# aalto-speech/AaltoASR

Measured on AMD Instinct MI355X. Metric: frames/sec GMM log-lik (39-d, 50k Gauss) + MFCC, 1/2/4/8 MI355X, higher is better.
Workload: dtype f32 (2-term fp16 split on the matrix cores, f32 accumulate); 1 GPU; configs[2]: full MFCC chain (FFT -> mel -> log -> DCT -> delta/delta-delta, CMS, normalisation) + 50000-Gaussian scoring + 2-byte LNA codes on 1 h of synthetic 16 kHz audio as 360 x 10 s utterances (449280 frames), int16 samples resident in HBM; dim=39, gaussians=50000, states=3125, gpus_flag=1

## Files before the change

### aaltoasr_amd/capi.py

```python
from __future__ import annotations

import ctypes as C
import os
import re
from typing import Optional

import numpy as np

HERE = os.path.dirname(os.path.abspath(__file__))
LIB_PATH = os.path.join(os.environ.get("AASR_LIBDIR") or os.path.join(HERE, "lib"), "libaasr.so")
HEADER_PATH = os.path.join(HERE, "..", "include", "aasr.h")

AASR_OK = 0
AASR_ERR_INVALID = -1
AASR_ERR_UNSUPPORTED = -2
AASR_ERR_NO_DEVICE = -3
AASR_ERR_IO = -4
AASR_ERR_SHORT_AUDIO = -5


class AasrError(RuntimeError):
    def __init__(self, code: int, msg: str):
        super().__init__("aasr status %d: %s" % (code, msg))
        self.code = code
# ... 596 lines not shown
        out = np.empty((n_frames, dim), dtype)
        fn = lib().aasr_feat_run if dtype == np.float32 else lib().aasr_feat_run_f64
        check(fn(self._h, _ptr(pcm), len(pcm), first_frame, n_frames,
                 module.encode() if module else None, _ptr(out)))
        return out

    def run_features(self, frames: np.ndarray, first_frame: int, n_frames: int,
                     module: Optional[str] = None, dtype=np.float32) -> np.ndarray:
        frames = np.ascontiguousarray(frames, np.float32)
        dim = self.module_dim(module) if module else self.dim
        out = np.empty((n_frames, dim), dtype)
        fn = lib().aasr_feat_run_features if dtype == np.float32 else lib().aasr_feat_run_features_f64
        check(fn(self._h, _ptr(frames), frames.size, first_frame, n_frames,
                 module.encode() if module else None, _ptr(out)))
        return out

    def run_batch_dev(self, d_pcm, pcm_off: np.ndarray, frame_off: np.ndarray, d_out, stream=None):
        pcm_off = np.ascontiguousarray(pcm_off, np.int64)
        frame_off = np.ascontiguousarray(frame_off, np.int64)
        check(lib().aasr_feat_run_batch_dev(self._h, _ptr(d_pcm), _ptr(pcm_off), _ptr(frame_off),
                                            len(pcm_off) - 1, _ptr(d_out), _stream_handle(stream)))

    def set_parameters(self, module: str, block_text: str) -> None:
        check(lib().aasr_feat_set_parameters(self._h, module.encode(), block_text.encode()))

    def get_parameters(self, module: str) -> str:
        out = C.c_void_p()
        n = C.c_int64()
        check(lib().aasr_feat_get_parameters(self._h, module.encode(), C.byref(out), C.byref(n)))
        try:
            return C.string_at(out, n.value).decode()
        finally:
            lib().aasr_free(out)

    def modules(self):
        L = lib()
        return [(L.aasr_feat_module_name(self._h, i).decode(), L.aasr_feat_module_type(self._h, i).decode())
                for i in range(L.aasr_feat_num_modules(self._h))]


def recipe_batch_range(total: int, num_batches: int, batch_index: int):
    f, n = C.c_int32(), C.c_int32()
    check(lib().aasr_recipe_batch_range(total, num_batches, batch_index, C.byref(f), C.byref(n)))
    return f.value, n.value


def debug_feat_fusion(on: bool) -> None:
    L = lib()
    L.aasr_debug_feat_fusion.argtypes = [C.c_int]
    L.aasr_debug_feat_fusion.restype = None
    L.aasr_debug_feat_fusion(int(on))


def debug_cluster_heap(on: bool) -> None:
    L = lib()
    L.aasr_debug_cluster_heap.argtypes = [C.c_int]
    L.aasr_debug_cluster_heap.restype = None
    L.aasr_debug_cluster_heap(int(on))


def recipe_frame_limits(start_time: float, end_time: float, frame_rate: float):
    a, b = C.c_int32(), C.c_int32()
    lib().aasr_recipe_frame_limits(start_time, end_time, frame_rate, C.byref(a), C.byref(b))
    return a.value, b.value


def recipe_read(text, num_batches: int = 0, batch_index: int = 0):
    out = C.c_void_p()
    n = C.c_int64()
    raw = text if isinstance(text, bytes) else text.encode()
    check(lib().aasr_recipe_read(raw, num_batches, batch_index, C.byref(out), C.byref(n)))
    try:
        table = C.string_at(out, n.value)
    finally:
        lib().aasr_free(out)
    rows = []
    for line in table.split(b"\n")[:-1]:
        f = line.split(b"\x1f")
        rows.append(tuple(x.decode("latin-1") for x in f[:4]) +
                    (float(np.float32(float(f[4]))), float(np.float32(float(f[5])))))
    return rows


def recipe_read_all(text, num_batches: int = 0, batch_index: int = 0, cluster_speakers: bool = False):
    out = C.c_void_p()
    n = C.c_int64()
    raw = text if isinstance(text, bytes) else text.encode()
    check(lib().aasr_recipe_read_all(raw, num_batches, batch_index, int(cluster_speakers), C.byref(out), C.byref(n)))
    try:
        table = C.string_at(out, n.value)
    finally:
        lib().aasr_free(out)
    rows = []
    for line in table.split(b"\n")[:-1]:
        f = [x.decode("latin-1") for x in line.split(b"\x1f")]
        rows.append(tuple(f[:7]) + (float(np.float32(float(f[7]))), float(np.float32(float(f[8]))),
                                    int(f[9]), int(f[10]), f[11], f[12]))
    return rows


def lna_read_file(path: str):
    out = C.POINTER(C.c_float)()
    S = C.c_int32()
    nb = C.c_int32()
    F = C.c_int64()
    check(lib().aasr_lna_read_file(path.encode(), C.byref(S), C.byref(nb), C.byref(F), C.byref(out)))
# ... 548 lines not shown
```

### aaltoasr_amd/csrc/feat_kernels.hip

```cpp
#include <hip/hip_runtime.h>

#include <cmath>
#include <cstring>
#include <climits>

#include "feat.h"

namespace aasr {

struct DevBatch {
  int n_utts;
  const int64_t *frame_off;
  const int64_t *pcm_off;
  const int32_t *first;
  const int32_t *eof_frame;
};

__device__ __forceinline__ int find_utt(const DevBatch &b, int64_t r, int span) {
  int lo = 0, hi = b.n_utts - 1;
  while (lo < hi) {
    int mid = (lo + hi + 1) >> 1;
    int64_t key = b.frame_off[mid] + (int64_t)mid * span;
    if (key <= r) lo = mid; else hi = mid - 1;
  }
  return lo;
}

__device__ __forceinline__ int find_utt_near(const DevBatch &b, int64_t r, int span, int64_t rows) {
  const int n = b.n_utts;
  int u = (int)((float)r * (float)n / (float)rows);
  u = u < 0 ? 0 : (u > n - 1 ? n - 1 : u);
  int lo = 0, hi = n - 1;
  for (int step = 0; step < 3; step++) {
    const int64_t k0 = b.frame_off[u] + (int64_t)u * span;
    const int64_t k1 = b.frame_off[u + 1] + (int64_t)(u + 1) * span;
    if (k0 > r && u > 0) {
      hi = u - 1;
      u--;
    } else if (k1 <= r && u < n - 1) {
      lo = u + 1;
      u++;
    } else {
      return u;
    }
  }
  while (lo < hi) {
    int mid = (lo + hi + 1) >> 1;
    int64_t key = b.frame_off[mid] + (int64_t)mid * span;
    if (key <= r) lo = mid; else hi = mid - 1;
  }
  return lo;
}

struct SrcMap {
// ... 188 lines not shown
  for (int q1 = 0, k = u; q1 < pr; q1++, k += m) scratch[q1] = F[k];
  for (int q1 = 0, k = u; q1 < pr; q1++, k += m) {
    int twidx = 0;
    cpx acc = scratch[0];
    for (int q = 1; q < pr; q++) {
      twidx += fstride * k;
      if (twidx >= n) twidx -= n;
      const cpx t = cmul(scratch[q], tw[twidx]);
      acc.r += t.r;
      acc.i += t.i;
    }
    F[k] = acc;
  }
}

__device__ __forceinline__ float glibc_logf(float x) {
  const double T[16][2] = {
      {0x1.661ec79f8f3bep+0, -0x1.57bf7808caadep-2}, {0x1.571ed4aaf883dp+0, -0x1.2bef0a7c06ddbp-2},
      {0x1.49539f0f010bp+0, -0x1.01eae7f513a67p-2},  {0x1.3c995b0b80385p+0, -0x1.b31d8a68224e9p-3},
      {0x1.30d190c8864a5p+0, -0x1.6574f0ac07758p-3}, {0x1.25e227b0b8eap+0, -0x1.1aa2bc79c81p-3},
      {0x1.1bb4a4a1a343fp+0, -0x1.a4e76ce8c0e5ep-4}, {0x1.12358f08ae5bap+0, -0x1.1973c5a611cccp-4},
      {0x1.0953f419900a7p+0, -0x1.252f438e10c1ep-5}, {0x1p+0, 0x0p+0},
      {0x1.e608cfd9a47acp-1, 0x1.aa5aa5df25984p-5},  {0x1.ca4b31f026aap-1, 0x1.c5e53aa362eb4p-4},
      {0x1.b2036576afce6p-1, 0x1.526e57720db08p-3},  {0x1.9c2d163a1aa2dp-1, 0x1.bc2860d22477p-3},
      {0x1.886e6037841edp-1, 0x1.1058bc8a07ee1p-2},  {0x1.767dcf5534862p-1, 0x1.4043057b6ee09p-2}};
  const double Ln2 = 0x1.62e42fefa39efp-1;
  const double A0 = -0x1.00ea348b88334p-2, A1 = 0x1.5575b0be00b6ap-2, A2 = -0x1.ffffef20a4123p-2;
  const uint32_t ix = __float_as_uint(x);
  if (ix == 0x3f800000u) return 0.0f;
  if (ix - 0x00800000u >= 0x7f800000u - 0x00800000u) return (float)log((double)x);
  const uint32_t tmp = ix - 0x3f330000u;
  const int i = (int)((tmp >> 19) & 15u);
  const int k = (int32_t)tmp >> 23;
  const uint32_t iz = ix - (tmp & 0xff800000u);
  const double z = (double)__uint_as_float(iz);
  const double r = z * T[i][0] - 1.0;
  const double y0 = T[i][1] + (double)k * Ln2;
  const double r2 = r * r;
  double y = A1 * r + A2;
  y = A0 * r2 + y;
  y = y * r2 + (y0 + r);
  return (float)y;
}

__device__ __forceinline__ float spec_value(float re, float im, int magnitude, int take_log) {
  float a = re * re;
  float c = im * im;
  float v = a + c;
  if (magnitude) v = (float)sqrt((double)v);
  if (take_log) v = glibc_logf(v);
  return v;
}

__device__ __forceinline__ void real_split(const cpx *buf, int nc, int k, const cpx *__restrict__ stw,
                                           float &re_k, float &im_k, float &re_n, float &im_n) {
  cpx fpk = buf[k], fpnk, f1k, f2k, t;
  fpnk.r = buf[nc - k].r;
  fpnk.i = -buf[nc - k].i;
  f1k.r = fpk.r + fpnk.r;  f1k.i = fpk.i + fpnk.i;
  f2k.r = fpk.r - fpnk.r;  f2k.i = fpk.i - fpnk.i;
  t = cmul(f2k, stw[k - 1]);
  float ar = f1k.r + t.r, ai = f1k.i + t.i, br = f1k.r - t.r, bi = t.i - f1k.i;
  re_k = ar * .5f;
  im_k = ai * .5f;
  re_n = br * .5f;
  im_n = bi * .5f;
}

template <bool FROM_PCM, bool GEN>
__global__ __launch_bounds__(256) void k_fft(DevBatch b, const int16_t *__restrict__ pcm,
                                             AudioPrm ap, const double *__restrict__ src,
                                             SrcMap sm, int L, int R, int64_t rows, FftPrm fp,
                                             double *__restrict__ dst) {
  extern __shared__ __attribute__((aligned(16))) char smem_raw[];
  const int wave = threadIdx.x >> 6, lane = threadIdx.x & 63;
  const int64_t r = (int64_t)blockIdx.x * 4 + wave;
  if (r >= rows) return;
  cpx *buf = (cpx *)smem_raw + (size_t)wave * fp.nc;
  const int nc = fp.nc, width = 2 * nc;

  const int16_t *p = nullptr;
  int64_t nsamp = 0, ws = 0;
  const double *xrow = nullptr;
  if (FROM_PCM) {
    int u = find_utt(b, r, L + R);
    int frame = b.first[u] - L + (int)(r - (b.frame_off[u] + (int64_t)u * (L + R)));
    ws = window_start(b, u, frame, ap);
    p = pcm + b.pcm_off[u];
    nsamp = b.pcm_off[u + 1] - b.pcm_off[u];
  } else {
    xrow = src + src_row(b, r, L + R, sm) * width;
  }
  for (int o = lane; o < nc; o += 64) {
    int s = fp.perm[o];
    double x0, x1;
    if (FROM_PCM) {
      x0 = (double)preemph_sample(p, nsamp, ws + 2 * s, ap.emph);
      x1 = (double)preemph_sample(p, nsamp, ws + 2 * s + 1, ap.emph);
    } else {
      x0 = xrow[2 * s];
      x1 = xrow[2 * s + 1];
    }
    cpx v;
    v.r = (float)((double)fp.hamming[2 * s] * x0);
    v.i = (float)((double)fp.hamming[2 * s + 1] * x1);
    buf[o] = v;
  }
  __builtin_amdgcn_fence(__ATOMIC_RELEASE, "wavefront");
  __builtin_amdgcn_wave_barrier();

  const cpx *tw = (const cpx *)fp.twiddle;
  for (int s = fp.ns - 1; s >= 0; s--) {
    const int pr = fp.radix[s], m = fp.sublen[s];
    const int fstride = fp.fstride[s];
    const int nb = fstride * m;
    if (GEN && pr > 5) {
      for (int bi = lane; bi < nb; bi += 64) kiss_butterfly_generic(buf, bi, pr, m, fstride, tw);
    } else {
      for (int bi = lane; bi < nb; bi += 64) kiss_butterfly(buf, bi, pr, m, fp.sub_magic[s], fstride, tw);
// ... 203 lines not shown
        power = power + v0;
        power = power + v1;
        power = power + v2;
        power = power + v3;
        power = power + v4;
        power = power + v5;
        power = power + v6;
        power = power + v7;
      }
      for (; i < nbins; i++) power = power + sf[i];
      if (r0 + ff < rows && !AASR_FDBG(128)) dst[(r0 + ff) * out_dim + sp.dct_dim] = log((double)power + 1e-10);
    }
    for (int slot = l; slot < (AASR_FDBG(4) ? 0 : sp.mel_dim); slot += TPF) {
      const int bin = t_mord[slot];
      float val = 0;
      const int e_end = t_moff[bin + 1];
      int e = t_moff[bin];
      for (; e + 4 <= e_end; e += 4) {
        const double p0 = (double)t_msc[e] * (double)spec[t_mt[e]];
        const double p1 = (double)t_msc[e + 1] * (double)spec[t_mt[e + 1]];
        const double p2 = (double)t_msc[e + 2] * (double)spec[t_mt[e + 2]];
        const double p3 = (double)t_msc[e + 3] * (double)spec[t_mt[e + 3]];
        val = (float)((double)val + p0);
        val = (float)((double)val + p1);
        val = (float)((double)val + p2);
        val = (float)((double)val + p3);
      }
      for (; e < e_end; e++) val = (float)((double)val + (double)t_msc[e] * (double)spec[t_mt[e]]);
      const float q = (float)((double)val / (double)t_msum[bin]);
      double o;
      if (sp.mel_root) {
        o = pow((double)q, 0.1);
      } else {
        const float a = q + 1.0f;
        o = (double)glibc_logf(a);
      }
      melv[(size_t)f * sp.mel_dim + bin] = o;
    }
    __builtin_amdgcn_fence(__ATOMIC_RELEASE, "wavefront");
    __builtin_amdgcn_wave_barrier();
    if (r0 + f < rows && !AASR_FDBG(128)) {
      const double *data = melv + (size_t)f * sp.mel_dim;
      for (int i = l; i < sp.dct_dim; i += TPF) {
        double acc = 0.0;
        if (sp.zeroth && i == 0) {
          for (int k = 0; k < sp.mel_dim; k++) acc += data[k];
        } else {
          const spec_tbl_t *c = t_dct + (size_t)(i - (sp.zeroth ? 1 : 0)) * sp.mel_dim;
#pragma unroll 4
          for (int k = 0; k < sp.mel_dim; k++) acc += data[k] * (double)c[k];
        }
        dst[(r0 + f) * out_dim + i] = acc;
      }
    }
    __builtin_amdgcn_fence(__ATOMIC_RELEASE, "wavefront");
    __builtin_amdgcn_wave_barrier();
  }
}

struct TemporalPrm {
  int dx, w1, w2;
  float norm1, norm2;
  const float *mean, *scale;
  const float *matrix, *bias;
  int dim;
};

#ifdef AASR_TR
constexpr int kTemporalRows = AASR_TR;
#else
constexpr int kTemporalRows = 64;
#endif

static inline size_t temporal_smem(int tile_rows, int dx, int H, int w2, int dim) {
  return (size_t)(tile_rows + 2 * H) * dx * 8 + (size_t)(tile_rows + 2 * w2) * dx * 8 + (size_t)tile_rows * 3 * dx * 8 + 16 +
         (size_t)(3 * dx) * ((dim + 2) / 3) * 16 + (size_t)(6 * dx + dim) * 4;
}

template <int ROWS, int NT>
__global__ __launch_bounds__(NT) void k_temporal_fused(DevBatch b, const double *__restrict__ src,
                                                        SrcMap sm, int span, int64_t rows,
                                                        TemporalPrm tp, int dbg, double *__restrict__ dst) {
  extern __shared__ __attribute__((aligned(16))) char smem_raw[];
  const int dx = tp.dx, H = tp.w1 + tp.w2, md = 3 * tp.dx;
  const unsigned dx_magic = fast_magic(dx), dim_magic = fast_magic(tp.dim);
  double *xs = (double *)smem_raw;
  double *d1 = xs + (size_t)(ROWS + 2 * H) * dx;
  double *nrm = d1 + (size_t)(ROWS + 2 * tp.w2) * dx;
  float4 *mt = (float4 *)(smem_raw + ((((size_t)(2 * ROWS + 2 * H + 2 * tp.w2) * dx + (size_t)ROWS * md) * 8 + 15) & ~(size_t)15));
  const int ngrp = (tp.dim + 2) / 3;
  const unsigned ngrp_magic = fast_magic(ngrp);
  if (tp.matrix && !AASR_FDBG(8))
    for (int e = threadIdx.x; e < md * ngrp; e += NT) {
      const int j = fast_div(e, ngrp_magic), g = e - j * ngrp;
      float4 v;
      v.x = tp.matrix[(size_t)(3 * g) * md + j];
      v.y = 3 * g + 1 < tp.dim ? tp.matrix[(size_t)(3 * g + 1) * md + j] : 0.0f;
      v.z = 3 * g + 2 < tp.dim ? tp.matrix[(size_t)(3 * g + 2) * md + j] : 0.0f;
      v.w = 0.0f;
      mt[e] = v;
    }
  float *nmean = (float *)(mt + (size_t)md * ngrp), *nscale = nmean + md, *nbias = nscale + md;
  for (int e = threadIdx.x; e < md; e += NT) {
    nmean[e] = tp.mean[e];
    nscale[e] = tp.scale[e];
  }
// ... 383 lines not shown
  const double *data = src + src_row(b, r, span, sm) * src_dim;
  const float *w = coef + (size_t)i * stride;
  double t = 0;
  for (int j = 0, fi = start[i]; j < len[i]; j++, fi++) t += data[fi * frame_dim + d] * (double)w[j];
  const float v = (float)t;
  dst[idx] = (v < 0.0f) ? 0.0f : v;
}

__global__ void k_vtln_linear(DevBatch b, const double *__restrict__ src, SrcMap sm, int span,
                              int64_t rows, int dim, const float *__restrict__ bins,
                              double *__restrict__ dst) {
  int64_t idx = (int64_t)blockIdx.x * blockDim.x + threadIdx.x;
  if (idx >= rows * dim) return;
  int64_t r = idx / dim;
  int bi = (int)(idx - r * dim);
  const double *data = src + src_row(b, r, span, sm) * dim;
  const float pos = bins[bi];
  const float p = ceilf(pos) - pos;
  const float q = 1 - p;
  const double lo = (double)p * data[(int)floorf(pos)];
  const double hi = (double)q * data[(int)ceilf(pos)];
  dst[idx] = lo + hi;
}

__global__ void k_quanteq(DevBatch b, const double *__restrict__ src, SrcMap sm, int span,
                          int64_t rows, int dim, const float *__restrict__ alpha,
                          const float *__restrict__ gamma, const float *__restrict__ qmax,
                          double *__restrict__ dst) {
  int64_t idx = (int64_t)blockIdx.x * blockDim.x + threadIdx.x;
  if (idx >= rows * dim) return;
  int64_t r = idx / dim;
  int k = (int)(idx - r * dim);
  const double x = src[src_row(b, r, span, sm) * dim + k];
  if (!alpha) {
    dst[idx] = x;
    return;
  }
  const double ratio = x / (double)qmax[k];
  const float one_minus = 1 - alpha[k];
  const double ex = (double)gamma[k] + (double)one_minus * ratio;
  dst[idx] = (double)qmax[k] * ((double)alpha[k] * pow(ratio, ex));
}

template <class T>
__global__ void k_emit(const double *__restrict__ src, int64_t n, T *__restrict__ dst) {
  int64_t idx = (int64_t)blockIdx.x * blockDim.x + threadIdx.x;
  if (idx < n) dst[idx] = (T)src[idx];
}


static inline unsigned grid_for(int64_t n) { return (unsigned)((n + 255) / 256); }

static int g_feat_fusion = AASR_EXPERIMENT_ENV("AASR_FEAT_FUSE") ? atoi(AASR_EXPERIMENT_ENV("AASR_FEAT_FUSE")) : 1;

void feat_run_batch(aasr_feat *h, const int16_t *d_pcm, const UttBatch &ub, int target,
                    float *out_f32, double *out_f64, hipStream_t stream) {
  const int nm = (int)h->mods.size();
  const int n = ub.n_utts;
  if (n <= 0) return;
  const int64_t total = ub.frame_off[n];
  if (total <= 0) return;
  const FeatModule &base = h->mods[0];

  std::vector<int> L(nm, -1), R(nm, -1), consumers(nm, 0);
  L[target] = R[target] = 0;
  for (int i = target; i >= 0; i--) {
    if (L[i] < 0) continue;
    const FeatModule &m = h->mods[i];
    for (int s : m.sources) {
      L[s] = std::max(L[s], L[i] + m.own_left + m.lead_left);
      R[s] = std::max(R[s], R[i] + m.own_right);
      consumers[s]++;
    }
  }

  std::vector<int32_t> eof(n);
  for (int u = 0; u < n; u++) {
    int64_t ns = ub.pcm_off[u + 1] - ub.pcm_off[u];
    if (base.type == MOD_PRE) {
      if ((ub.pcm_off[u] & 1) || ns / 2 / base.dim < 1)
        raise(AASR_ERR_SHORT_AUDIO, "PreModule: Could not read the file");
      eof[u] = (int32_t)(ns / 2 / base.dim);
      continue;
    }
    if (ns < base.width + 1)
      raise(AASR_ERR_SHORT_AUDIO, "audio shorter than frame");
    if (ns > INT32_MAX)
      raise(AASR_ERR_UNSUPPORTED, "utterance longer than 2^31 samples");
    eof[u] = feat_eof_frame(h, ns);
    if (eof[u] < 1) raise(AASR_ERR_SHORT_AUDIO, "audio shorter than frame");
  }
  const size_t stage_bytes = (size_t)(n + 1) * 16 + (size_t)n * 8;
  if (h->stage_event && h->stage_busy) {
    AASR_HIP(hipEventSynchronize(h->stage_event));
    h->stage_busy = false;
  }
  if (stage_bytes > h->stage_cap) {
    if (h->stage_host) (void)hipHostFree(h->stage_host);
    h->stage_host = nullptr;
    AASR_HIP(hipHostMalloc(&h->stage_host, stage_bytes * 2, hipHostMallocDefault));
    h->stage_cap = stage_bytes * 2;
  }
  if (!h->stage_event) AASR_HIP(hipEventCreateWithFlags(&h->stage_event, hipEventDisableTiming));
  {
    char *sp = (char *)h->stage_host;
    int64_t *s_fo = (int64_t *)sp;
    int64_t *s_po = s_fo + (n + 1);
    int32_t *s_first = (int32_t *)(s_po + (n + 1));
    int32_t *s_eof = s_first + n;
    memcpy(s_fo, ub.frame_off.data(), (n + 1) * sizeof(int64_t));
    memcpy(s_po, ub.pcm_off.data(), (n + 1) * sizeof(int64_t));
    memcpy(s_first, ub.first.data(), n * sizeof(int32_t));
    memcpy(s_eof, eof.data(), n * sizeof(int32_t));
    h->d_desc.ensure(stage_bytes);
// ... 47 lines not shown
      if (h->mods[A].dim != dx || h->mods[B].dim != dx || Cm.dim != 3 * dx || T.src_dim != 3 * dx) continue;
      if ((int)h->mods[N].mean.size() != 3 * dx || (int)h->mods[N].scale.size() != 3 * dx) continue;
      const int H = h->mods[A].delta_width + h->mods[B].delta_width;
      constexpr int TR = kTemporalRows;
      if (temporal_smem(TR, dx, H, h->mods[B].delta_width, T.dim) > 64 * 1024) continue;
      tgX = X; tgA = A; tgB = B; tgN = N; tgT = ti;
      skip[A] = skip[B] = skip[C] = skip[N] = 1;
    }
  }

  auto rows_of = [&](int i) { return total + (int64_t)n * (L[i] + R[i]); };
  auto map_of = [&](int i, int s) {
    return SrcMap{(L[s] + R[s]) - (L[i] + R[i]), L[s] - L[i]};
  };

  bool emitted = false;
  for (int i = 0; i <= target; i++) {
    if (L[i] < 0 || skip[i]) continue;
    FeatModule &m = h->mods[i];
    const int64_t rows = rows_of(i);
    const int span = L[i] + R[i];
    if (i == sgG) {
      const FeatModule &F = h->mods[sgF], &M = h->mods[sgM], &D = h->mods[sgD];
      SpectralPrm sp;
      sp.fp.nc = F.fft.nc;
      sp.fp.ns = F.fft.ns;
      for (int k = 0; k < 16; k++) {
        sp.fp.radix[k] = F.fft.radix[k];
        sp.fp.sublen[k] = F.fft.sublen[k];
        sp.fp.sub_magic[k] = fast_magic(F.fft.sublen[k]);
        sp.fp.fstride[k] = k < F.fft.ns ? F.fft.nc / (F.fft.radix[k] * F.fft.sublen[k]) : 0;
      }
      sp.fp.hamming = F.fft.hamming.p;
      sp.fp.twiddle = F.fft.twiddle.p;
      sp.fp.stwiddle = F.fft.stwiddle.p;
      sp.fp.perm = F.fft.perm.p;
      sp.fp.magnitude = F.magnitude;
      sp.fp.take_log = F.take_log;
      sp.mel_dim = M.dim;
      sp.mel_root = M.root;
      sp.mel_off = M.mel_off.p;
      sp.mel_t = M.mel_t.p;
      sp.mel_scale = M.mel_scale.p;
      sp.mel_sum = M.mel_sum.p;
      sp.mel_order = M.mel_order.p;
      sp.dct_dim = D.dim;
      sp.zeroth = D.zeroth;
      sp.dct_cos = D.dct_cos.p;
      sp.mel_terms = (int)M.mel_t.n;
      const SpectralLds lds(F.fft.nc, M.dim, sp.mel_terms, D.dim - (D.zeroth ? 1 : 0));
      const int64_t nblk = (rows + SPEC_FRAMES - 1) / SPEC_FRAMES;
      const int passes = (int)std::max<int64_t>(1, std::min<int64_t>(8, nblk / 4096));
      h->bufs[i].ensure((size_t)rows * m.dim);
      hipLaunchKernelGGL(k_spectral_fused, dim3((unsigned)((nblk + passes - 1) / passes)), dim3(256), lds.total,
                         stream, db, d_pcm, ap, L[i], R[i], rows, sp, passes,
                         AASR_EXPERIMENT_ENV("AASR_SPEC_DBG") ? atoi(AASR_EXPERIMENT_ENV("AASR_SPEC_DBG")) : 0, h->bufs[i].p);
      AASR_HIP(hipGetLastError());
      continue;
    }
    if (i == tgT) {
      const FeatModule &A = h->mods[tgA], &B = h->mods[tgB], &N = h->mods[tgN];
      TemporalPrm tp;
      tp.dx = h->mods[tgX].dim;
      tp.w1 = A.delta_width;
      tp.w2 = B.delta_width;
      tp.norm1 = A.delta_norm;
      tp.norm2 = B.delta_norm;
      tp.mean = N.d_mean.p;
      tp.scale = N.d_scale.p;
      tp.matrix = m.matrix_defined ? m.d_matrix.p : nullptr;
      tp.bias = m.bias_defined ? m.d_bias.p : nullptr;
      tp.dim = m.dim;
      constexpr int TR = kTemporalRows;
      const int H = tp.w1 + tp.w2;
      const size_t smem = temporal_smem(TR, tp.dx, H, tp.w2, m.dim);
      h->bufs[i].ensure((size_t)rows * m.dim);
      constexpr int TNT = TR >= 128 ? 1024 : TR >= 64 ? 512 : 256;
      if (smem > 64 * 1024)
        AASR_HIP(hipFuncSetAttribute((const void *)k_temporal_fused<TR, TNT>, hipFuncAttributeMaxDynamicSharedMemorySize, (int)smem));
      hipLaunchKernelGGL((k_temporal_fused<TR, TNT>), dim3((unsigned)((rows + TR - 1) / TR)), dim3(TNT), smem, stream, db,
                         (const double *)h->bufs[tgX].p, map_of(i, tgX), span, rows, tp,
                         AASR_EXPERIMENT_ENV("AASR_TEMP_DBG") ? atoi(AASR_EXPERIMENT_ENV("AASR_TEMP_DBG")) : 0, h->bufs[i].p);
      AASR_HIP(hipGetLastError());
      continue;
    }
    if (m.type == MOD_AUDIOFILE && i != target && consumers[0] == 1) {
      bool only_fft = false;
      for (int j = 1; j <= target; j++)
        if (L[j] >= 0 && h->mods[j].type == MOD_FFT && h->mods[j].sources[0] == 0) only_fft = true;
      if (only_fft) continue;
    }
    h->bufs[i].ensure((size_t)rows * m.dim);
    double *dst = h->bufs[i].p;
    const int s0 = m.sources.empty() ? -1 : m.sources[0];
    const double *src = s0 >= 0 ? h->bufs[s0].p : nullptr;
    SrcMap sm = s0 >= 0 ? map_of(i, s0) : SrcMap{0, 0};
    const int64_t nelem = rows * m.dim;
    switch (m.type) {
      case MOD_PRE:
        hipLaunchKernelGGL(k_pre_frames, dim3(grid_for(nelem)), dim3(256), 0, stream, db,
                           (const float *)d_pcm, m.dim, L[i], R[i], rows, dst);
        break;
      case MOD_AUDIOFILE:
        hipLaunchKernelGGL(k_audio_frames, dim3(grid_for(nelem)), dim3(256), 0, stream, db, d_pcm,
                           ap, L[i], R[i], rows, dst);
        break;
      case MOD_FFT: {
        FftPrm fp;
        fp.nc = m.fft.nc;
// ... 151 lines not shown
        AASR_HIP(hipMemcpy(dst, hout.data(), hout.size() * sizeof(double), hipMemcpyHostToDevice));
        break;
      }
      case MOD_MEAN_SUBTRACTOR: {
        const int ms_dbg = AASR_EXPERIMENT_ENV("AASR_CMS_DBG") ? atoi(AASR_EXPERIMENT_ENV("AASR_CMS_DBG")) : 0;
        auto smem_of = [&](int tile_rows) {
          const size_t n = (size_t)(tile_rows + kCmsLead + m.cms_left + m.cms_right);
          return (n + n / 8 + 1) * m.dim * 8;
        };
        int tile_rows = 0;
        if (smem_of(128) <= 78 * 1024) tile_rows = 128;
        else if (smem_of(64) <= 52 * 1024) tile_rows = 64;
        else if (smem_of(128) <= 156 * 1024) tile_rows = 128;
        else if (smem_of(64) <= 156 * 1024) tile_rows = 64;
        const bool emit_f32 = i == target && g_feat_fusion && out_f32 && !out_f64;
        auto launch = [&](auto kern, int rows_per, int nt, auto *out) {
          const size_t smem = smem_of(rows_per);
          if (smem > 64 * 1024)
            AASR_HIP(hipFuncSetAttribute((const void *)kern, hipFuncAttributeMaxDynamicSharedMemorySize, (int)smem));
          hipLaunchKernelGGL(kern, dim3((unsigned)((rows + rows_per - 1) / rows_per)), dim3(nt), smem, stream, db, src, sm,
                             span, L[i], rows, m.dim, m.cms_left, m.cms_right, ms_dbg, out);
        };
        if (tile_rows >= 128) {
          if (emit_f32) launch(k_mean_subtract_tiled<128, float, 512>, 128, 512, out_f32);
          else launch(k_mean_subtract_tiled<128, double, 512>, 128, 512, dst);
          emitted = emit_f32;
        } else if (tile_rows > 0) {
          if (emit_f32) launch(k_mean_subtract_tiled<64, float, 256>, 64, 256, out_f32);
          else launch(k_mean_subtract_tiled<64, double, 256>, 64, 256, dst);
          emitted = emit_f32;
        } else {
          hipLaunchKernelGGL(k_mean_subtract, dim3(grid_for(nelem)), dim3(256), 0, stream, db, src,
                             sm, span, rows, m.dim, m.cms_left, m.cms_right, dst);
        }
        break;
      }
    }
    AASR_HIP(hipGetLastError());
  }
  const int64_t nout = total * h->mods[target].dim;
  if (emitted) return;
  if (out_f32)
    hipLaunchKernelGGL(k_emit<float>, dim3(grid_for(nout)), dim3(256), 0, stream,
                       (const double *)h->bufs[target].p, nout, out_f32);
  if (out_f64)
    hipLaunchKernelGGL(k_emit<double>, dim3(grid_for(nout)), dim3(256), 0, stream,
                       (const double *)h->bufs[target].p, nout, out_f64);
  AASR_HIP(hipGetLastError());
}

}

extern "C" void aasr_debug_feat_fusion(int on) { aasr::g_feat_fusion = on; }
```

### include/aasr.h

```cpp
#ifndef AASR_H
#define AASR_H

#include <stddef.h>
#include <stdint.h>

#ifdef __cplusplus
extern "C" {
#endif

typedef int aasr_status;
enum {
  AASR_OK = 0,
  AASR_ERR_INVALID = -1,
  AASR_ERR_UNSUPPORTED = -2,
  AASR_ERR_NO_DEVICE = -3,
  AASR_ERR_IO = -4,
  AASR_ERR_SHORT_AUDIO = -5
};

typedef struct aasr_feat aasr_feat;
typedef struct aasr_gmm aasr_gmm;

const char *aasr_last_error(void);
const char *aasr_version(void);
int aasr_device_count(void);
aasr_status aasr_set_device(int ordinal);


aasr_status aasr_feat_create(const char *cfg_text, aasr_feat **out);
void aasr_feat_destroy(aasr_feat *h);

int aasr_feat_dim(const aasr_feat *h);
float aasr_feat_frame_rate(const aasr_feat *h);
int aasr_feat_sample_rate(const aasr_feat *h);
int aasr_feat_module_dim(const aasr_feat *h, const char *module_name);
void aasr_feat_halo(const aasr_feat *h, int *left, int *right);

int aasr_feat_last_frame(const aasr_feat *h, int64_t n_samples);
int aasr_feat_eof_frame(const aasr_feat *h, int64_t n_samples);

aasr_status aasr_feat_run_features(aasr_feat *h, const float *features, int64_t n_values,
                                   int32_t first_frame, int32_t n_frames,
                                   const char *module_name, float *out);
aasr_status aasr_feat_run_features_f64(aasr_feat *h, const float *features, int64_t n_values,
                                       int32_t first_frame, int32_t n_frames,
                                       const char *module_name, double *out);
aasr_status aasr_feat_write_config(const aasr_feat *h, char **text, int64_t *len);
int aasr_feat_input_is_features(const aasr_feat *h);
int aasr_feat_pre_legacy(const aasr_feat *h);
int aasr_feat_input_dim(const aasr_feat *h);

aasr_status aasr_feat_run(aasr_feat *h, const int16_t *pcm, int64_t n_samples,
                          int32_t first_frame, int32_t n_frames,
                          const char *module_name, float *out);
aasr_status aasr_feat_run_dev(aasr_feat *h, const int16_t *d_pcm,
                              int64_t n_samples, int32_t first_frame,
                              int32_t n_frames, float *d_out, void *stream);
aasr_status aasr_feat_run_f64(aasr_feat *h, const int16_t *pcm,
                              int64_t n_samples, int32_t first_frame,
                              int32_t n_frames, const char *module_name,
                              double *out);

aasr_status aasr_feat_run_f64_dev(aasr_feat *h, const int16_t *d_pcm, int64_t n_samples,
                                  int32_t first_frame, int32_t n_frames, double *d_out,
                                  void *stream);

aasr_status aasr_feat_run_batch_dev(aasr_feat *h, const int16_t *d_pcm,
                                    const int64_t *pcm_off,
                                    const int64_t *frame_off, int32_t n_utts,
                                    float *d_out, void *stream);

aasr_status aasr_feat_set_parameters(aasr_feat *h, const char *module_name,
                                     const char *params_text);
aasr_status aasr_feat_get_parameters(const aasr_feat *h, const char *module_name, char **text,
                                     int64_t *len);
int aasr_feat_num_modules(const aasr_feat *h);
const char *aasr_feat_module_name(const aasr_feat *h, int index);
const char *aasr_feat_module_type(const aasr_feat *h, int index);


aasr_status aasr_gmm_create_diag(int32_t dim, int32_t num_gaussians,
                                 const double *mean, const double *var,
                                 int32_t num_states, const int32_t *mix_off,
                                 const int32_t *mix_idx, const double *mix_w,
                                 aasr_gmm **out);
aasr_status aasr_gmm_create_full(int32_t dim, int32_t num_gaussians,
                                 const double *mean, const double *cov,
                                 int32_t num_states, const int32_t *mix_off,
                                 const int32_t *mix_idx, const double *mix_w,
                                 aasr_gmm **out);
aasr_status aasr_gmm_create_from_files(const char *gk_path, const char *mc_path,
                                       const char *ph_path, aasr_gmm **out);
aasr_status aasr_gmm_write_cache(const aasr_gmm *h, const char *cache_path);
aasr_status aasr_gmm_create_from_cache(const char *cache_path, aasr_gmm **out);
aasr_status aasr_gmm_create_from_cache_checked(const char *cache_path, const char *gk_path,
                                               const char *mc_path, const char *ph_path,
                                               aasr_gmm **out);
void aasr_gmm_destroy(aasr_gmm *h);

int32_t aasr_gmm_mixture_size(const aasr_gmm *h, int32_t state);
aasr_status aasr_gmm_mixture_get(const aasr_gmm *h, int32_t state, int32_t *index, double *weight);
aasr_status aasr_gmm_gaussian_get(const aasr_gmm *h, int32_t gaussian, double *mean, double *var);

int aasr_gmm_dim(const aasr_gmm *h);
int aasr_gmm_num_states(const aasr_gmm *h);
int aasr_gmm_num_gaussians(const aasr_gmm *h);
int64_t aasr_gmm_expanded_rows(const aasr_gmm *h);

aasr_status aasr_gmm_set_cmllr(aasr_gmm *h, int32_t n_transforms,
                               const int32_t *gauss_to_transform, const double *W);

aasr_status aasr_gmm_read_clustering(aasr_gmm *h, const char *gcl_path);
aasr_status aasr_gmm_set_clustering(aasr_gmm *h, int32_t n_clusters, int64_t n_pairs,
                                    const int32_t *gauss_index, const int32_t *cluster_index);
aasr_status aasr_gmm_set_clustering_min_evals(aasr_gmm *h, double min_clusters,
                                              double min_gaussians);
int32_t aasr_gmm_num_clusters(const aasr_gmm *h);

enum { AASR_PREC_F32 = 0, AASR_PREC_F64 = 1, AASR_PREC_F32_CENTRED = 2, AASR_PREC_BF16X3 = 3, AASR_PREC_F16X2 = 4 };
aasr_status aasr_gmm_set_precision(aasr_gmm *h, int prec);
int aasr_gmm_get_precision(const aasr_gmm *h);
int aasr_gmm_effective_precision(const aasr_gmm *h);
aasr_status aasr_gmm_precision_states(const aasr_gmm *h, int64_t *states_f16x2, int64_t *states_probe_moved);
// ... 304 lines not shown
```

Before: 44.06 million frames/s.

## Add compile-time specialised spectral kernel for 128-point FFT, 21 mel, 12 DCT

Adds a templated spectral kernel specialised for a 256-sample real FFT (nc=128, radix 4-4-4-2), 21 mel bins and 12 cepstra. It keeps twiddles, mel and DCT tables in LDS and holds butterflies in registers with a padded LDS layout. It fully unrolls the mel and DCT loops and dispatches to this kernel when the configuration matches, otherwise using the generic fused kernel. The aim is to cut generic loop overhead, global table reads and bank conflicts in MFCC front-end work, at the cost of more code and a path that only covers one configuration.

```diff
diff --git a/aaltoasr_amd/capi.py b/aaltoasr_amd/capi.py
--- a/aaltoasr_amd/capi.py
+++ b/aaltoasr_amd/capi.py
@@ -672,6 +672,20 @@
     L.aasr_debug_feat_fusion(int(on))
 
 
+def debug_feat_fixed(on: bool) -> None:
+    L = lib()
+    L.aasr_debug_feat_fixed.argtypes = [C.c_int]
+    L.aasr_debug_feat_fixed.restype = None
+    L.aasr_debug_feat_fixed(int(on))
+
+
+def debug_feat_last_spectral() -> int:
+    L = lib()
+    L.aasr_debug_feat_last_spectral.argtypes = []
+    L.aasr_debug_feat_last_spectral.restype = C.c_int32
+    return int(L.aasr_debug_feat_last_spectral())
+
+
 def debug_cluster_heap(on: bool) -> None:
     L = lib()
     L.aasr_debug_cluster_heap.argtypes = [C.c_int]
diff --git a/aaltoasr_amd/csrc/feat_kernels.hip b/aaltoasr_amd/csrc/feat_kernels.hip
--- a/aaltoasr_amd/csrc/feat_kernels.hip
+++ b/aaltoasr_amd/csrc/feat_kernels.hip
@@ -1,5 +1,6 @@
 #include <hip/hip_runtime.h>
 
+#include <atomic>
 #include <cmath>
 #include <cstring>
 #include <climits>
@@ -294,19 +295,23 @@
   return v;
 }
 
-__device__ __forceinline__ void real_split(const cpx *buf, int nc, int k, const cpx *__restrict__ stw,
-                                           float &re_k, float &im_k, float &re_n, float &im_n) {
-  cpx fpk = buf[k], fpnk, f1k, f2k, t;
-  fpnk.r = buf[nc - k].r;
-  fpnk.i = -buf[nc - k].i;
+__device__ __forceinline__ void real_split_values(cpx bk, cpx bn, cpx w, float &re_k, float &im_k, float &re_n,
+                                                  float &im_n) {
+  cpx fpk = bk, fpnk, f1k, f2k, t;
+  fpnk.r = bn.r;
+  fpnk.i = -bn.i;
   f1k.r = fpk.r + fpnk.r;  f1k.i = fpk.i + fpnk.i;
   f2k.r = fpk.r - fpnk.r;  f2k.i = fpk.i - fpnk.i;
-  t = cmul(f2k, stw[k - 1]);
+  t = cmul(f2k, w);
   float ar = f1k.r + t.r, ai = f1k.i + t.i, br = f1k.r - t.r, bi = t.i - f1k.i;
   re_k = ar * .5f;
   im_k = ai * .5f;
   re_n = br * .5f;
   im_n = bi * .5f;
+}
+__device__ __forceinline__ void real_split(const cpx *buf, int nc, int k, const cpx *__restrict__ stw,
+                                           float &re_k, float &im_k, float &re_n, float &im_n) {
+  real_split_values(buf[k], buf[nc - k], stw[k - 1], re_k, im_k, re_n, im_n);
 }
 
 template <bool FROM_PCM, bool GEN>
@@ -616,6 +621,254 @@
         }
         dst[(r0 + f) * out_dim + i] = acc;
       }
+    }
+    __builtin_amdgcn_fence(__ATOMIC_RELEASE, "wavefront");
+    __builtin_amdgcn_wave_barrier();
+  }
+}
+
+struct SpecFixedPlan {
+  static constexpr int nc = 128, ns = 4;
+  static constexpr int radix[4] = {4, 4, 4, 2}, sublen[4] = {32, 8, 2, 1};
+};
+
+template <int NC, int MELDIM, int DCTDIM>
+struct SpecFixedLds {
+  static constexpr int a16(int n) { return (n + 15) & ~15; }
+  static constexpr int buf_stride = NC + NC / 8;
+  static constexpr int spec_stride = (NC + 1) | 3;
+  static constexpr int bufs = 0;
+  static constexpr int spec = bufs + a16(SPEC_FRAMES * buf_stride * 8);
+  static constexpr int melv = spec + a16(SPEC_FRAMES * spec_stride * 4);
+  static constexpr int tw = melv + a16(SPEC_FRAMES * MELDIM * 8);
+  static constexpr int stw = tw + a16(NC * 8);
+  static constexpr int moff = stw + a16(NC / 2 * 8);
+  static constexpr int msum = moff + a16((MELDIM + 1) * 4);
+  static constexpr int mord = msum + a16(MELDIM * 4);
+  static constexpr int dct = mord + a16(MELDIM * 4);
+  static constexpr int prm = dct + a16(DCTDIM * MELDIM * 4);
+  static constexpr int mt = prm + a16(SPEC_FRAMES * 3 * 8);
+  static __host__ __device__ int msc(int mel_terms) { return mt + a16(mel_terms * 4); }
+  static __host__ __device__ int total(int mel_terms) { return mt + 2 * a16(mel_terms * 4); }
+};
+
+template <int NC, int MELDIM, int DCTDIM>
+__global__ __launch_bounds__(256) void k_spectral_fixed(DevBatch b, const int16_t *__restrict__ pcm, AudioPrm ap, int L,
+                                                        int R, int64_t rows, SpectralPrm sp, int passes, int dbg,
+                                                        double *__restrict__ dst) {
+  static_assert(NC == SpecFixedPlan::nc && SPEC_TPF == 16 && NC == 8 * SPEC_TPF, "the stage shapes below are those of nc = 128");
+  static_assert(DCTDIM <= SPEC_TPF, "one DCT round");
+  extern __shared__ __attribute__((aligned(16))) char smem_raw[];
+  constexpr int FB = SPEC_FRAMES, TPF = SPEC_TPF, nbins = NC + 1;
+  typedef SpecFixedLds<NC, MELDIM, DCTDIM> lds;
+  cpx *bufs = (cpx *)(smem_raw + lds::bufs);
+  float *specs = (float *)(smem_raw + lds::spec);
+  double *melv = (double *)(smem_raw + lds::melv);
+  cpx *t_tw = (cpx *)(smem_raw + lds::tw);
+  cpx *t_stw = (cpx *)(smem_raw + lds::stw);
+  int32_t *t_moff = (int32_t *)(smem_raw + lds::moff);
+  float *t_msum = (float *)(smem_raw + lds::msum);
+  int32_t *t_mord = (int32_t *)(smem_raw + lds::mord);
+  float *t_dct = (float *)(smem_raw + lds::dct);
+  int64_t *s_prm = (int64_t *)(smem_raw + lds::prm);
+  int32_t *t_mt = (int32_t *)(smem_raw + lds::mt);
+  float *t_msc = (float *)(smem_raw + lds::msc(sp.mel_terms));
+  const int tid = threadIdx.x;
+  const int f = tid / TPF, l = tid - f * TPF;
+
+  for (int i = tid; i < NC; i += 256) t_tw[i] = ((const cpx *)sp.fp.twiddle)[i];
+  for (int i = tid; i < NC / 2; i += 256) t_stw[i] = ((const cpx *)sp.fp.stwiddle)[i];
+  for (int i = tid; i <= MELDIM; i += 256) t_moff[i] = sp.mel_off[i];
+  for (int i = tid; i < sp.mel_terms; i += 256) {
+    t_mt[i] = sp.mel_t[i];
+    t_msc[i] = sp.mel_scale[i];
+  }
+  for (int i = tid; i < MELDIM; i += 256) {
+    t_msum[i] = sp.mel_sum[i];
+    t_mord[i] = sp.mel_order[i];
+  }
+  for (int i = tid; i < DCTDIM * MELDIM; i += 256) t_dct[i] = sp.dct_cos[i];
+
+  const int sb = 2 * ((l >> 2) + 4 * (l & 3));
+  auto soff = [](int q) { return 32 * (q >> 1) + 128 * (q & 1); };
+  float ham[16];
+#pragma unroll
+  for (int q = 0; q < 8; q++) {
+    ham[2 * q] = sp.fp.hamming[sb + soff(q)];
+    ham[2 * q + 1] = sp.fp.hamming[sb + soff(q) + 1];
+  }
+
+  cpx *buf = bufs + f * lds::buf_stride;
+  float *spec = specs + f * lds::spec_stride;
+  constexpr int out_dim = DCTDIM + 1;
+  const int64_t nblk = (rows + FB - 1) / FB;
+  int u_cur = -1;
+  for (int pass = 0; pass < passes; pass++) {
+    const int64_t blk = (int64_t)blockIdx.x * passes + pass;
+    if (blk >= nblk) break;
+    const int64_t r0 = blk * FB;
+    __syncthreads();
+    if (tid < FB) {
+      int64_t r = r0 + tid;
+      if (r > rows - 1) r = rows - 1;
+      int u;
+      if (AASR_FDBG(1)) {
+        u = 0;
+      } else if (u_cur < 0) {
+        u = find_utt_near(b, r, L + R, rows);
+      } else {
+        u = u_cur;
+        while (u + 1 < b.n_utts && b.frame_off[u + 1] + (int64_t)(u + 1) * (L + R) <= r) u++;
+      }
+      u_cur = u;
+      const int frame = b.first[u] - L + (int)(r - (b.frame_off[u] + (int64_t)u * (L + R)));
+      s_prm[3 * tid] = window_start(b, u, frame, ap);
+      s_prm[3 * tid + 1] = b.pcm_off[u];
+      s_prm[3 * tid + 2] = b.pcm_off[u + 1] - b.pcm_off[u];
+    }
+    __syncthreads();
+    cpx x[8];
+#pragma unroll
+    for (int q = 0; q < 8; q++) x[q].r = x[q].i = 0.0f;
+    if (!(AASR_FDBG(32) || AASR_FDBG(8))) {
+      const int64_t ws = s_prm[3 * f], ns = s_prm[3 * f + 2];
+      const int16_t *p = pcm + s_prm[3 * f + 1];
+      const bool inside = ws >= 0 && ws + 2 * NC < ns;
+      if (inside) {
+        const int16_t *pq = p + ws + sb;
+#pragma unroll
+        for (int q = 0; q < 8; q++) {
+          const float c0 = (float)pq[soff(q)], c1 = (float)pq[soff(q) + 1], c2 = (float)pq[soff(q) + 2];
+          const float p0 = ap.emph * c0, p1 = ap.emph * c1;
+          x[q].r = ham[2 * q] * (c1 - p0);
+          x[q].i = ham[2 * q + 1] * (c2 - p1);
+        }
+      } else {
+#pragma unroll
+        for (int q = 0; q < 8; q++) {
+          const int64_t i = ws + sb + soff(q);
+          const float c0 = (i >= 0 && i < ns) ? (float)p[i] : 0.0f;
+          const float c1 = (i + 1 >= 0 && i + 1 < ns) ? (float)p[i + 1] : 0.0f;
+          const float c2 = (i + 2 >= 0 && i + 2 < ns) ? (float)p[i + 2] : 0.0f;
+          const float p0 = ap.emph * c0, p1 = ap.emph * c1;
+          x[q].r = ham[2 * q] * (c1 - p0);
+          x[q].i = ham[2 * q + 1] * (c2 - p1);
+        }
+      }
+    }
+    if (!AASR_FDBG(2)) {
+      const cpx w0 = t_tw[0];
+#pragma unroll
+      for (int bq = 0; bq < 4; bq++) bfly2_values(x[2 * bq], x[2 * bq + 1], w0);
+      bfly4_values(x[0], x[2], x[4], x[6], w0, w0, w0);
+      bfly4_values(x[1], x[3], x[5], x[7], t_tw[16], t_tw[32], t_tw[48]);
+    }
+#pragma unroll
+    for (int q = 0; q < 8; q++) buf[9 * l + q] = x[q];
+    __builtin_amdgcn_fence(__ATOMIC_RELEASE, "wavefront");
+    __builtin_amdgcn_wave_barrier();
+    if (!AASR_FDBG(2)) {
+      {
+        cpx *F = buf + 36 * (l >> 2) + (l & 3);
+        const int j4 = 4 * (l & 3);
+#pragma unroll
+        for (int r = 0; r < 2; r++) {
+          cpx f0 = F[4 * r], f1 = F[4 * r + 9], f2 = F[4 * r + 18], f3 = F[4 * r + 27];
+          bfly4_values(f0, f1, f2, f3, t_tw[j4 + 16 * r], t_tw[2 * j4 + 32 * r], t_tw[3 * j4 + 48 * r]);
+          F[4 * r] = f0;
+          F[4 * r + 9] = f1;
+          F[4 * r + 18] = f2;
+          F[4 * r + 27] = f3;
+        }
+      }
+      __builtin_amdgcn_fence(__ATOMIC_RELEASE, "wavefront");
+      __builtin_amdgcn_wave_barrier();
+      {
+        cpx *F = buf + l + (l >> 3);
+#pragma unroll
+        for (int r = 0; r < 2; r++) {
+          cpx f0 = F[18 * r], f1 = F[18 * r + 36], f2 = F[18 * r + 72], f3 = F[18 * r + 108];
+          bfly4_values(f0, f1, f2, f3, t_tw[l + 16 * r], t_tw[2 * l + 32 * r], t_tw[3 * l + 48 * r]);
+          F[18 * r] = f0;
+          F[18 * r + 36] = f1;
+          F[18 * r + 72] = f2;
+          F[18 * r + 108] = f3;
+        }
+      }
+      __builtin_amdgcn_fence(__ATOMIC_RELEASE, "wavefront");
+      __builtin_amdgcn_wave_barrier();
+    }
+    if (!AASR_FDBG(64)) {
+      if (l == 0) {
+        const cpx t0 = buf[0];
+        spec[0] = spec_value(t0.r + t0.i, 0.0f, 0, 0);
+        spec[NC] = spec_value(t0.r - t0.i, 0.0f, 0, 0);
+      }
+#pragma unroll
+      for (int r = 0; r < NC / 2 / TPF; r++) {
+        const int k = (r == 0 && l == 0) ? NC / 2 : l + TPF * r, kn = NC - k;
+        float re_k, im_k, re_n, im_n;
+        real_split_values(buf[k + (k >> 3)], buf[kn + (kn >> 3)], t_stw[k - 1], re_k, im_k, re_n, im_n);
+        if (k != kn) spec[k] = spec_value(re_k, im_k, 0, 0);
+        spec[kn] = spec_value(re_n, im_n, 0, 0);
+      }
+    }
+    __syncthreads();
+    if ((tid >> 6) == (pass & 3) && (tid & 63) < FB && !AASR_FDBG(16)) {
+      const int ff = tid & 63;
+      const float *sf = specs + ff * lds::spec_stride;
+      float power = 0;
+#pragma unroll 2
+      for (int i = 0; i + 8 <= nbins; i += 8) {
+        const float v0 = sf[i], v1 = sf[i + 1], v2 = sf[i + 2], v3 = sf[i + 3];
+        const float v4 = sf[i + 4], v5 = sf[i + 5], v6 = sf[i + 6], v7 = sf[i + 7];
+        power = power + v0;
+        power = power + v1;
+        power = power + v2;
+        power = power + v3;
+        power = power + v4;
+        power = power + v5;
+        power = power + v6;
+        power = power + v7;
+      }
+#pragma unroll
+      for (int i = nbins & ~7; i < nbins; i++) power = power + sf[i];
+      if (r0 + ff < rows && !AASR_FDBG(128)) dst[(r0 + ff) * out_dim + DCTDIM] = log((double)power + 1e-10);
+    }
+    if (!AASR_FDBG(4)) {
+#pragma unroll
+      for (int slot0 = 0; slot0 < MELDIM; slot0 += TPF) {
+        const int slot = slot0 + l;
+        if (slot0 + TPF > MELDIM && slot >= MELDIM) break;
+        const int bin = t_mord[slot];
+        float val = 0;
+        const int e_end = t_moff[bin + 1];
+        int e = t_moff[bin];
+        for (; e + 4 <= e_end; e += 4) {
+          const double p0 = (double)t_msc[e] * (double)spec[t_mt[e]];
+          const double p1 = (double)t_msc[e + 1] * (double)spec[t_mt[e + 1]];
+          const double p2 = (double)t_msc[e + 2] * (double)spec[t_mt[e + 2]];
+          const double p3 = (double)t_msc[e + 3] * (double)spec[t_mt[e + 3]];
+          val = (float)((double)val + p0);
+          val = (float)((double)val + p1);
+          val = (float)((double)val + p2);
+          val = (float)((double)val + p3);
+        }
+        for (; e < e_end; e++) val = (float)((double)val + (double)t_msc[e] * (double)spec[t_mt[e]]);
+        const float q = (float)((double)val / (double)t_msum[bin]);
+        const float a = q + 1.0f;
+        melv[f * MELDIM + bin] = (double)glibc_logf(a);
+      }
+    }
+    __builtin_amdgcn_fence(__ATOMIC_RELEASE, "wavefront");
+    __builtin_amdgcn_wave_barrier();
+    if (r0 + f < rows && l < DCTDIM && !AASR_FDBG(128)) {
+      const double *data = melv + f * MELDIM;
+      const float *c = t_dct + l * MELDIM;
+      double acc = 0.0;
+#pragma unroll
+      for (int k = 0; k < MELDIM; k++) acc += data[k] * (double)c[k];
+      dst[(r0 + f) * out_dim + l] = acc;
     }
     __builtin_amdgcn_fence(__ATOMIC_RELEASE, "wavefront");
     __builtin_amdgcn_wave_barrier();
@@ -1105,6 +1358,18 @@
 static inline unsigned grid_for(int64_t n) { return (unsigned)((n + 255) / 256); }
 
 static int g_feat_fusion = AASR_EXPERIMENT_ENV("AASR_FEAT_FUSE") ? atoi(AASR_EXPERIMENT_ENV("AASR_FEAT_FUSE")) : 1;
+static std::atomic<int> g_feat_fixed{AASR_EXPERIMENT_ENV("AASR_FEAT_FIXED") ? atoi(AASR_EXPERIMENT_ENV("AASR_FEAT_FIXED")) : 1};
+static std::atomic<int> g_feat_last_spectral{0};
+
+constexpr int kSpecFixedMel = 21, kSpecFixedDct = 12;
+static bool spec_fixed_matches(const FeatModule &F, const FeatModule &M, const FeatModule &D) {
+  if (F.fft.nc != SpecFixedPlan::nc || F.fft.ns != SpecFixedPlan::ns) return false;
+  for (int st = 0; st < SpecFixedPlan::ns; st++)
+    if (F.fft.radix[st] != SpecFixedPlan::radix[st] || F.fft.sublen[st] != SpecFixedPlan::sublen[st]) return false;
+  if (F.magnitude || F.take_log || M.root || D.zeroth) return false;
+  if (M.dim != kSpecFixedMel || D.dim != kSpecFixedDct) return false;
+  return SpecFixedLds<SpecFixedPlan::nc, kSpecFixedMel, kSpecFixedDct>::total((int)M.mel_t.n) <= 64 * 1024;
+}
 
 void feat_run_batch(aasr_feat *h, const int16_t *d_pcm, const UttBatch &ub, int target,
                     float *out_f32, double *out_f64, hipStream_t stream) {
@@ -1113,6 +1378,7 @@
   if (n <= 0) return;
   const int64_t total = ub.frame_off[n];
   if (total <= 0) return;
+  g_feat_last_spectral = 0;
   const FeatModule &base = h->mods[0];
 
   std::vector<int> L(nm, -1), R(nm, -1), consumers(nm, 0);
@@ -1266,9 +1532,19 @@
       const int64_t nblk = (rows + SPEC_FRAMES - 1) / SPEC_FRAMES;
       const int passes = (int)std::max<int64_t>(1, std::min<int64_t>(8, nblk / 4096));
       h->bufs[i].ensure((size_t)rows * m.dim);
-      hipLaunchKernelGGL(k_spectral_fused, dim3((unsigned)((nblk + passes - 1) / passes)), dim3(256), lds.total,
-                         stream, db, d_pcm, ap, L[i], R[i], rows, sp, passes,
-                         AASR_EXPERIMENT_ENV("AASR_SPEC_DBG") ? atoi(AASR_EXPERIMENT_ENV("AASR_SPEC_DBG")) : 0, h->bufs[i].p);
+      const int spec_dbg = AASR_EXPERIMENT_ENV("AASR_SPEC_DBG") ? atoi(AASR_EXPERIMENT_ENV("AASR_SPEC_DBG")) : 0;
+      const dim3 grid((unsigned)((nblk + passes - 1) / passes));
+      if (g_feat_fixed && spec_fixed_matches(F, M, D)) {
+        typedef SpecFixedLds<SpecFixedPlan::nc, kSpecFixedMel, kSpecFixedDct> flds;
+        hipLaunchKernelGGL((k_spectral_fixed<SpecFixedPlan::nc, kSpecFixedMel, kSpecFixedDct>), grid, dim3(256),
+                           (size_t)flds::total(sp.mel_terms), stream, db, d_pcm, ap, L[i], R[i], rows, sp, passes, spec_dbg,
+                           h->bufs[i].p);
+        g_feat_last_spectral = 2;
+      } else {
+        hipLaunchKernelGGL(k_spectral_fused, grid, dim3(256), lds.total, stream, db, d_pcm, ap, L[i], R[i], rows, sp,
+                           passes, spec_dbg, h->bufs[i].p);
+        g_feat_last_spectral = 1;
+      }
       AASR_HIP(hipGetLastError());
       continue;
     }
@@ -1526,3 +1802,5 @@
 }
 
 extern "C" void aasr_debug_feat_fusion(int on) { aasr::g_feat_fusion = on; }
+extern "C" void aasr_debug_feat_fixed(int on) { aasr::g_feat_fixed = on; }
+extern "C" int32_t aasr_debug_feat_last_spectral(void) { return aasr::g_feat_last_spectral; }
diff --git a/include/aasr.h b/include/aasr.h
--- a/include/aasr.h
+++ b/include/aasr.h
@@ -69,6 +69,9 @@
                                     const int64_t *pcm_off,
                                     const int64_t *frame_off, int32_t n_utts,
                                     float *d_out, void *stream);
+
+void aasr_debug_feat_fixed(int on);
+int32_t aasr_debug_feat_last_spectral(void);
 
 aasr_status aasr_feat_set_parameters(aasr_feat *h, const char *module_name,
                                      const char *params_text);
```

Result: faster. 45.05 million frames/s (median of 6 runs) (+2.3%).
